# aaryaamoharir/ImageTransformations

Hardware: AMD Instinct MI355X
Metric: Mpixels/sec, 5x5 Gaussian + bilinear rotate on 4K RGB; % HBM roofline (higher is better)
Workload: dtype u8/f32

## Files before the change

imagetransformations_amd/csrc/affine.hip:

```cpp
#include "imgxf_common.h"
#include "pixel_ops.h"
#include <math.h>
#include <algorithm>
#include <string.h>
#include <stdlib.h>

namespace imgxf {

struct AffineParams {
    double m[6];
    int fx[6];
    int64_t q0, q3;
    int64_t q1, q4;
    int64_t x00, y00;
    u32 ntx_magic;
    int sx[4], sy[4];
    u8 fill[4];
    int strip_w;
};

struct FastArith {
    typedef float T;
    static __device__ __forceinline__ T mul(T a, T b) { return a * b; }
    static __device__ __forceinline__ T add(T a, T b) { return a + b; }
// ... 1026 lines not shown

}
#include "affine_mf.inc"
#include "affine_wq.inc"
namespace imgxf {

constexpr int BILINEAR_TALL_NOT_TAKEN = 1 << 30;

template <int BHT, int PITCH, int MAXROWS>
static int launch_bilinear_tall(const View& s, const View& d, const AffineParams& Pin, const View& dbg, const double* m,
                                int bw, int bh, int ntx, bool pr, hipStream_t st) {
    const AffineParams& P = Pin;
    const int bwt = (int)ceil(fabs(m[0]) * 31 + fabs(m[1]) * (BHT - 1)) + 4;
    const int bht = (int)ceil(fabs(m[3]) * 31 + fabs(m[4]) * (BHT - 1)) + 4;
    const int ntyt = (d.h + BHT - 1) / BHT;
    if (bwt > PITCH || bht > MAXROWS || bw > PITCH || (int64_t)ntx * ntyt * ntx >= ((int64_t)1 << 32))
        return BILINEAR_TALL_NOT_TAKEN;
    const bool want_f32 = dbg.p != nullptr;
    const int fpb = knob_int(K_AFFINE_FPB, 16);
    const int afpb = fpb;
    const bool mf = BHT == MF_TILE_H && !want_f32 && afpb >= 2 && d.n >= 2 && bht <= 64 &&
                    (int64_t)d.h * d.rs < ((int64_t)1 << 32);
    const int nch = (bwt * 3 + 15 + 15) / 16;
    const bool dma = mf && !knob_set(K_AFFINE_NO_DMA) && bht <= 52 && bwt <= 52 && 52 * nch <= 768 &&
                     ((((uintptr_t)s.p) | (uintptr_t)s.rs | (uintptr_t)s.fs) & 15) == 0 && s.w * 3 >= 16 &&
                     (int64_t)s.h * s.rs < ((int64_t)1 << 32);
    if (mf && !knob_set(K_AFFINE_NO_DMA)) {
        const int bwq = (int)ceil(fabs(m[0]) * 31 + fabs(m[1]) * 15) + 4, bhq = (int)ceil(fabs(m[3]) * 31 + fabs(m[4]) * 15) + 4;
        const int nchq = (bwq * 3 + 15 + 15) / 16;
        const int ntxq = (d.w + 127) / 128, ntyq = (d.h + 15) / 16;
        const bool aligned = ((((uintptr_t)s.p) | (uintptr_t)s.rs | (uintptr_t)s.fs | ((uintptr_t)d.p) | (uintptr_t)d.rs | (uintptr_t)d.fs) & 15) == 0 &&
                             (d.w * 3) % 16 == 0 && s.w * 3 >= 16;
        if (aligned && bwq <= WQ_PITCH && bhq * nchq <= WQ_MAXCH && bhq * (WQ_PITCH / 4) <= 192 &&
            (int64_t)s.h * s.rs < ((int64_t)1 << 32) && (int64_t)ntxq * ntyq < ((int64_t)1 << 27)) {
            AffineParams Pq = Pin;
            Pq.strip_w = 0;
            const int fpbq = knob_int(K_AFFINE_FPB, 24);
            dim3 grid((unsigned)(ntxq * ntyq), (unsigned)((d.n + fpbq - 1) / fpbq));
            if (ntxq >= 8) { Pq.strip_w = (ntxq + 7) / 8; grid.x = (unsigned)(8 * Pq.strip_w * ntyq); }
            const size_t lds = (size_t)4 * ((size_t)bhq * WQ_PITCH * 4 + 2 * ((size_t)bhq * nchq * 16 + 64)) + 2 * 16 * 384;
            if (pr) hipLaunchKernelGGL((affine_bilinear_wq_kernel<true>), grid, dim3(256), lds, st, s, d, Pq, ntxq, ntyq, fpbq, nchq, bhq);
            else hipLaunchKernelGGL((affine_bilinear_wq_kernel<false>), grid, dim3(256), lds, st, s, d, Pq, ntxq, ntyq, fpbq, nchq, bhq);
            return launch_status();
        }
    }
    if (dma) {
        dim3 grid((unsigned)(ntx * ntyt), (unsigned)((d.n + afpb - 1) / afpb));
        AffineParams Ps = Pin;
        if (ntx >= 16) { Ps.strip_w = (ntx + 7) / 8; grid.x = (unsigned)(8 * Ps.strip_w * ntyt); }
        const size_t lds = (size_t)52 * 56 * 4 + 2 * ((size_t)52 * nch * 16 + 64);
        if (pr) hipLaunchKernelGGL((affine_bilinear_mf_kernel<true, 56, 13, true>), grid, dim3(256), lds, st, s, d, Ps, ntx, ntyt, fpb, nch);
        else hipLaunchKernelGGL((affine_bilinear_mf_kernel<false, 56, 13, true>), grid, dim3(256), lds, st, s, d, Ps, ntx, ntyt, fpb, nch);
        return launch_status();
    }
    TileList list;
    list.n = 0;
    const int64_t ax = 31 * P.q0, bx = (BHT - 1) * P.q1, ay = 31 * P.q3, by = (BHT - 1) * P.q4;
    const int64_t xlo_o = std::min(ax, (int64_t)0) + std::min(bx, (int64_t)0), xhi_o = std::max(ax, (int64_t)0) + std::max(bx, (int64_t)0);
    const int64_t ylo_o = std::min(ay, (int64_t)0) + std::min(by, (int64_t)0), yhi_o = std::max(ay, (int64_t)0) + std::max(by, (int64_t)0);
    for (int ty = 0; ty < ntyt && list.n <= BILINEAR_LIST_MAX; ++ty)
        for (int tx = 0; tx < ntx; ++tx) {
            const int64_t XT = P.x00 + (int64_t)(tx * 32) * P.q0 + (int64_t)(ty * BHT) * P.q1;
            const int64_t YT = P.y00 + (int64_t)(tx * 32) * P.q3 + (int64_t)(ty * BHT) * P.q4;
            const bool clean = (int)((XT + xlo_o) >> 40) >= 0 && (int)((YT + ylo_o) >> 40) >= 0 &&
                               (int)((XT + xhi_o) >> 40) + 1 <= s.w - 1 && (int)((YT + yhi_o) >> 40) + 1 <= s.h - 1 &&
                               tx * 32 + 32 <= d.w && ty * BHT + BHT <= d.h &&
                               !((int)((XT + xhi_o) >> 40) + 1 == s.w - 1 && (int)((YT + yhi_o) >> 40) + 1 == s.h - 1);
            if (!clean) {
                if (list.n < BILINEAR_LIST_MAX) list.idx[list.n] = (u32)(ty * ntx + tx);
                ++list.n;
            }
        }
    if (list.n > BILINEAR_LIST_MAX) return BILINEAR_TALL_NOT_TAKEN;
    if (list.n < ntx * ntyt && mf) {
        const dim3 grid((unsigned)(ntx * ntyt), (unsigned)((d.n + afpb - 1) / afpb));
        const size_t lds = (size_t)2 * PITCH * (bht <= 52 ? 52 : 64) * 4 + 16;
        if (bht <= 52) {
            if (pr) hipLaunchKernelGGL((affine_bilinear_mf_kernel<true, PITCH, 13, false>), grid, dim3(256), lds, st, s, d, P, ntx, ntyt, fpb, 0);
            else hipLaunchKernelGGL((affine_bilinear_mf_kernel<false, PITCH, 13, false>), grid, dim3(256), lds, st, s, d, P, ntx, ntyt, fpb, 0);
        } else {
            if (pr) hipLaunchKernelGGL((affine_bilinear_mf_kernel<true, PITCH, 16, false>), grid, dim3(256), lds, st, s, d, P, ntx, ntyt, fpb, 0);
            else hipLaunchKernelGGL((affine_bilinear_mf_kernel<false, PITCH, 16, false>), grid, dim3(256), lds, st, s, d, P, ntx, ntyt, fpb, 0);
        }
        IMGXF_CHECK(launch_status());
    } else if (list.n < ntx * ntyt) {
        const dim3 grid((unsigned)(ntx * ntyt), (unsigned)d.n);
        const size_t lds = (size_t)PITCH * bht * 4 + 16;
        if (pr && want_f32) hipLaunchKernelGGL((affine_bilinear_lds_interior_kernel<true, PITCH, true, BHT>), grid, dim3(256), lds, st, s, d, P, dbg, ntx, ntyt);
        else if (pr) hipLaunchKernelGGL((affine_bilinear_lds_interior_kernel<true, PITCH, false, BHT>), grid, dim3(256), lds, st, s, d, P, dbg, ntx, ntyt);
        else if (want_f32) hipLaunchKernelGGL((affine_bilinear_lds_interior_kernel<false, PITCH, true, BHT>), grid, dim3(256), lds, st, s, d, P, dbg, ntx, ntyt);
        else hipLaunchKernelGGL((affine_bilinear_lds_interior_kernel<false, PITCH, false, BHT>), grid, dim3(256), lds, st, s, d, P, dbg, ntx, ntyt);
        IMGXF_CHECK(launch_status());
    }
    if (list.n > 0) {
        const dim3 grid((unsigned)((BHT / 32) * list.n), (unsigned)d.n);
        const size_t lds = (size_t)PITCH * bh * 4 + 16;
        if (pr && want_f32) hipLaunchKernelGGL((affine_bilinear_lds_list_kernel<true, PITCH, true, BHT>), grid, dim3(256), lds, st, s, d, P, dbg, ntx, list);
        else if (pr) hipLaunchKernelGGL((affine_bilinear_lds_list_kernel<true, PITCH, false, BHT>), grid, dim3(256), lds, st, s, d, P, dbg, ntx, list);
        else if (want_f32) hipLaunchKernelGGL((affine_bilinear_lds_list_kernel<false, PITCH, true, BHT>), grid, dim3(256), lds, st, s, d, P, dbg, ntx, list);
        else hipLaunchKernelGGL((affine_bilinear_lds_list_kernel<false, PITCH, false, BHT>), grid, dim3(256), lds, st, s, d, P, dbg, ntx, list);
    }
    return launch_status();
}

int run_affine(const imgxf_view* src, const imgxf_view* dst, const double* m, int filter,
               const uint8_t* fill, int precise, const imgxf_view* dbg_f32, void* stream) {
    IMGXF_CHECK(check_view(src));
    IMGXF_CHECK(check_view(dst));
    if (!m) return IMGXF_ERR_NULL;
    if (src->n != dst->n || src->c != dst->c) return IMGXF_ERR_SHAPE;
    if (filter < 0 || filter > 2) return IMGXF_ERR_ARG;
    if (filter == IMGXF_FILTER_NEAREST && m[1] == 0.0 && m[3] == 0.0) return IMGXF_ERR_UNSUPPORTED;
    if (filter != IMGXF_FILTER_NEAREST && src->c == 4) return IMGXF_ERR_UNSUPPORTED;
    if (empty_view(dst)) return IMGXF_OK;
    if (empty_view(src)) return IMGXF_ERR_SHAPE;
    AffineParams P; memset(&P, 0, sizeof(P));
    for (int i = 0; i < 6; ++i) P.m[i] = m[i];
    affine_fixed_matrix(m, P.fx);
    if (fill) for (int j = 0; j < dst->c; ++j) P.fill[j] = fill[j];
    View dbg; memset(&dbg, 0, sizeof(dbg));
    if (dbg_f32) {
        IMGXF_CHECK(check_view(dbg_f32, 4));
        if (!same_geometry(dst, dbg_f32)) return IMGXF_ERR_SHAPE;
        dbg = make_view(dbg_f32);
    }
    const View s = make_view(src), d = make_view(dst);
    hipStream_t st = (hipStream_t)stream;
    const bool pr = precise != 0 || filter == IMGXF_FILTER_NEAREST;
    if (filter == IMGXF_FILTER_NEAREST && src->c == 3 && !knob_set(K_AFFINE_NO_LDS) &&
        ((((uintptr_t)src->data) | (uintptr_t)src->row_stride | (uintptr_t)src->frame_stride) & 3) == 0) {
        bool nowrap = true;
        for (int cy = 0; cy < 2; ++cy)
            for (int cx = 0; cx < 2; ++cx) {
                const double X = cx ? dst->w + 32 : 0, Y = cy ? dst->h + 32 : 0;
                const double xs = (double)P.fx[2] + (double)P.fx[1] * Y + (double)P.fx[0] * X;
                const double ys = (double)P.fx[5] + (double)P.fx[4] * Y + (double)P.fx[3] * X;
                if (fabs(xs) > 2.0e9 || fabs(ys) > 2.0e9) nowrap = false;
            }
        const int bw = (int)ceil((fabs((double)P.fx[0]) * 31 + fabs((double)P.fx[1]) * 31) / 65536.0) + 3;
        const int bh = (int)ceil((fabs((double)P.fx[3]) * 31 + fabs((double)P.fx[4]) * 31) / 65536.0) + 3;
        const int ntx = (d.w + 31) / 32, nty = (d.h + 31) / 32;
        if (nowrap && bw <= 97 && bh <= 100 && (int64_t)ntx * nty < 0x7fffffff && d.n <= 65535) {
            dim3 grid((unsigned)(ntx * nty), (unsigned)d.n);
            P.ntx_magic = (u32)((((uint64_t)1 << 32) + ntx - 1) / ntx);
            const bool no_dma = knob_set(K_AFFINE_NO_DMA);
            {
                const int bwq = (int)ceil((fabs((double)P.fx[0]) * 31 + fabs((double)P.fx[1]) * 15) / 65536.0) + 3;
                const int bhq = (int)ceil((fabs((double)P.fx[3]) * 31 + fabs((double)P.fx[4]) * 15) / 65536.0) + 3;
                const int nchq = (bwq * 3 + 15 + 15) / 16;
                const int kwq = (bhq * nchq + 63) / 64;
                const int ntxq = (d.w + 127) / 128, ntyq = (d.h + 15) / 16;
                const bool aligned = ((((uintptr_t)s.p) | (uintptr_t)s.rs | (uintptr_t)s.fs | ((uintptr_t)d.p) | (uintptr_t)d.rs | (uintptr_t)d.fs) & 15) == 0 &&
                                     (d.w * 3) % 16 == 0 && (s.w * 3) % 16 == 0 && s.w * 3 >= 16 &&
                                     (int64_t)s.h * s.rs < ((int64_t)1 << 32);
                if (aligned && !no_dma && kwq <= NQ_KW && (int64_t)ntxq * ntyq < ((int64_t)1 << 27)) {
                    AffineParams Pq = P;
                    Pq.strip_w = 0;
                    unsigned gx = (unsigned)(ntxq * ntyq);
                    const int fpbq = max(1, min(knob_int(K_AFFINE_FPB, 1), d.n));
                    const dim3 grid(gx, (unsigned)((d.n + fpbq - 1) / fpbq));
                    const size_t nbufq = fpbq > 1 ? 2 : 1;
                    const size_t lds = nbufq * ((size_t)4 * ((size_t)bhq * nchq * 16 + 16) + 16 * 384);
#define IMGXF_NQ_LAUNCH(KWV) hipLaunchKernelGGL((affine_nearest_wq_kernel<KWV>), grid, dim3(256), lds, st, s, d, Pq, ntxq, ntyq, fpbq, nchq, bhq)
                    switch (kwq) {
                        case 1: IMGXF_NQ_LAUNCH(1); break; case 2: IMGXF_NQ_LAUNCH(2); break; case 3: IMGXF_NQ_LAUNCH(3); break;
                        case 4: IMGXF_NQ_LAUNCH(4); break; case 5: IMGXF_NQ_LAUNCH(5); break; case 6: IMGXF_NQ_LAUNCH(6); break;
                        case 7: IMGXF_NQ_LAUNCH(7); break; default: IMGXF_NQ_LAUNCH(8); break;
                    }
#undef IMGXF_NQ_LAUNCH
                    return launch_status();
                }
            }
            if (bw <= 49 && bh <= 52 && !no_dma && src->w * 3 >= 16 && (src->w * 3) % 16 == 0 &&
                ((((uintptr_t)src->data) | (uintptr_t)src->row_stride | (uintptr_t)src->frame_stride) & 15) == 0) {
                const int bw64 = (int)ceil((fabs((double)P.fx[0]) * 31 + fabs((double)P.fx[1]) * 63) / 65536.0) + 3;
                const int bh64 = (int)ceil((fabs((double)P.fx[3]) * 31 + fabs((double)P.fx[4]) * 63) / 65536.0) + 3;
                const bool no_tall = knob_set(K_AFFINE_NO_TALL);
                if (bw64 <= 64 && bh64 <= 80 && !no_tall) {
                    const int nty64 = (d.h + 63) / 64;
                    unsigned gx = (unsigned)(ntx * nty64);
                    if (ntx >= 16) { P.strip_w = (ntx + 7) / 8; gx = (unsigned)(8 * P.strip_w * nty64); }
                    hipLaunchKernelGGL((affine_nearest_dma_kernel<64, 13>), dim3(gx, (unsigned)d.n), dim3(256),
                                       (size_t)13 * 16 * bh64 + 32, st, s, d, P, ntx, nty64);
                } else {
                    hipLaunchKernelGGL((affine_nearest_dma_kernel<32, 11>), grid, dim3(256), (size_t)11 * 16 * bh + 32, st, s, d, P, ntx, nty);
                }
                return launch_status();
            }
            if (bw <= 49) hipLaunchKernelGGL((affine_nearest_lds_kernel<49>), grid, dim3(256), (size_t)49 * bh * 4 + 16, st, s, d, P, ntx, nty);
            else if (bw <= 65) hipLaunchKernelGGL((affine_nearest_lds_kernel<65>), grid, dim3(256), (size_t)65 * bh * 4 + 16, st, s, d, P, ntx, nty);
            else hipLaunchKernelGGL((affine_nearest_lds_kernel<97>), grid, dim3(256), (size_t)97 * bh * 4 + 16, st, s, d, P, ntx, nty);
            return launch_status();
        }
    }
    bool fixed_ok = fabs(m[0]) < 64.0 && fabs(m[3]) < 64.0;
    for (int cy = 0; cy < 2 && fixed_ok; ++cy)
        for (int cx = 0; cx < 2; ++cx) {
            const double X = (cx ? dst->w + 4 : 0) + 0.5, Y = (cy ? dst->h : 0) + 0.5;
            const double xs = m[0] * X + m[1] * Y + m[2], ys = m[3] * X + m[4] * Y + m[5];
            if (!(fabs(xs) < 2097152.0 && fabs(ys) < 2097152.0)) fixed_ok = false;
        }
    P.q0 = fixed_ok ? llround(m[0] * 1099511627776.0) : 0;
    P.q3 = fixed_ok ? llround(m[3] * 1099511627776.0) : 0;
    fixed_ok = fixed_ok && fabs(m[1]) < 64.0 && fabs(m[4]) < 64.0;
    P.q1 = fixed_ok ? llround(m[1] * 1099511627776.0) : 0;
    P.q4 = fixed_ok ? llround(m[4] * 1099511627776.0) : 0;
    for (int k = 0; k < 4; ++k) {
        P.sx[k] = (int)((k * P.q0 + (k * P.q0 >= 0 ? 32768 : -32768)) / 65536);
        P.sy[k] = (int)((k * P.q3 + (k * P.q3 >= 0 ? 32768 : -32768)) / 65536);
    }
    if (fixed_ok) {
        const double x0d = (m[0] * 0.5 + m[1] * 0.5) + m[2] - 0.5, y0d = (m[3] * 0.5 + m[4] * 0.5) + m[5] - 0.5;
        P.x00 = (int64_t)floor(x0d * 1099511627776.0);
        P.y00 = (int64_t)floor(y0d * 1099511627776.0);
    }
    if (filter == IMGXF_FILTER_BILINEAR && (src->c == 1 || src->c == 3) && src->w >= 3 && src->h >= 2 && fixed_ok) {
        const bool no_lds = knob_set(K_AFFINE_NO_LDS);
        if (src->c == 3 && !no_lds &&
            ((((uintptr_t)src->data) | (uintptr_t)src->row_stride | (uintptr_t)src->frame_stride) & 3) == 0) {
            const int bw = (int)ceil(fabs(m[0]) * 31 + fabs(m[1]) * 31) + 4;
            const int bh = (int)ceil(fabs(m[3]) * 31 + fabs(m[4]) * 31) + 4;
            const int ntx = (d.w + 31) / 32, nty = (d.h + 31) / 32;
            if (bw <= 97 && bh <= 100 && (int64_t)ntx * nty < 0x7fffffff && d.n <= 65535) {
                dim3 grid((unsigned)(ntx * nty), (unsigned)d.n);
                P.ntx_magic = (u32)((((uint64_t)1 << 32) + ntx - 1) / ntx);
#define IMGXF_LDS_LAUNCH(KERNEL, PITCH, GRID, NTY, LDSB)                                            \
    do {                                                                                           \
        if (dbg.p) {                                                                               \
            if (pr) hipLaunchKernelGGL((KERNEL<true, PITCH, true>), GRID, dim3(256), LDSB, st, s, d, P, dbg, ntx, NTY); \
            else hipLaunchKernelGGL((KERNEL<false, PITCH, true>), GRID, dim3(256), LDSB, st, s, d, P, dbg, ntx, NTY); \
        } else {                                                                                   \
            if (pr) hipLaunchKernelGGL((KERNEL<true, PITCH, false>), GRID, dim3(256), LDSB, st, s, d, P, dbg, ntx, NTY); \
            else hipLaunchKernelGGL((KERNEL<false, PITCH, false>), GRID, dim3(256), LDSB, st, s, d, P, dbg, ntx, NTY); \
        }                                                                                          \
    } while (0)
#define IMGXF_LDS(PITCH)                                                                           \
    do {                                                                                           \
        const size_t lds = (size_t)PITCH * bh * 4 + 16;                                            \
        IMGXF_LDS_LAUNCH(affine_bilinear_lds_kernel, PITCH, grid, nty, lds);                       \
        return launch_status();                                                                    \
    } while (0)
                const bool no_tall = knob_set(K_AFFINE_NO_TALL);
                if (!no_tall) {
                    const int rc = launch_bilinear_tall<64, 49, 64>(s, d, P, dbg, m, bw, bh, ntx, pr, st);
                    if (rc != BILINEAR_TALL_NOT_TAKEN) return rc;
                }
                if (bw <= 49) IMGXF_LDS(49);
                if (bw <= 65) IMGXF_LDS(65);
                IMGXF_LDS(97);
#undef IMGXF_LDS
#undef IMGXF_LDS_LAUNCH
            }
        }
#define IMGXF_BIL(CC, PR, TXG, WX)                                                                 \
    do {                                                                                           \
        constexpr int BW = WX * TXG * 4, BH = (4 / WX) * (64 / TXG);                               \
        const int ntx = (d.w + BW - 1) / BW, nty = (d.h + BH - 1) / BH;                            \
        const int64_t nb = (int64_t)ntx * nty * d.n;                                               \
        if (nb > 0x7fffffff) return IMGXF_ERR_SHAPE;                                               \
        hipLaunchKernelGGL((affine_bilinear_kernel<CC, PR, TXG, WX>), dim3((unsigned)nb), dim3(256), 0, st, \
                           s, d, P, dbg, ntx, nty, (int)nb);                                       \
        return launch_status();                                                                    \
    } while (0)
        if (src->c == 3) {
            if (pr) IMGXF_BIL(3, true, 8, 2); else IMGXF_BIL(3, false, 8, 2);
        } else {
            if (pr) IMGXF_BIL(1, true, 8, 2); else IMGXF_BIL(1, false, 8, 2);
        }
#undef IMGXF_BIL
    }
    {
        const bool no_shear = knob_set(K_AFFINE_NO_SHEAR_FAST);
        const bool honly = m[3] == 0.0 && m[4] == 1.0 && m[5] == floor(m[5]) && fabs(m[5]) < 1.0e9;
        if (filter == IMGXF_FILTER_BICUBIC && honly && src->c == 3 && !dbg.p && !no_shear && src->w >= 4) {
            dim3 block(256), grid((unsigned)((d.w + 1023) / 1024), (unsigned)d.h, (unsigned)d.n);
            if (m[0] == 1.0) {
                if (pr) hipLaunchKernelGGL((shear_bicubic_kernel<true, true>), grid, block, 0, st, s, d, P);
                else hipLaunchKernelGGL((shear_bicubic_kernel<false, true>), grid, block, 0, st, s, d, P);
                IMGXF_CHECK(launch_status());
                hipLaunchKernelGGL(shear_edges_kernel, dim3((unsigned)((d.h * 8 + 255) / 256), (unsigned)d.n), dim3(256), 0, st, s, d, P);
                return launch_status();
            }
            if (pr) hipLaunchKernelGGL((shear_bicubic_kernel<true, false>), grid, block, 0, st, s, d, P);
            else hipLaunchKernelGGL((shear_bicubic_kernel<false, false>), grid, block, 0, st, s, d, P);
            return launch_status();
        }
    }
    switch (src->c) {
        case 1: return pr ? launch_affine_filter<1, PreciseArith>(filter, s, d, P, dbg, st)
                          : launch_affine_filter<1, FastArith>(filter, s, d, P, dbg, st);
        case 3: return pr ? launch_affine_filter<3, PreciseArith>(filter, s, d, P, dbg, st)
                          : launch_affine_filter<3, FastArith>(filter, s, d, P, dbg, st);
        case 4: return launch_affine_filter<4, PreciseArith>(filter, s, d, P, dbg, st);
        default: return IMGXF_ERR_UNSUPPORTED;
    }
}

__global__ void scale_tables_kernel(int* xtab, int* ytab, int* meta, int ow, int oh, int sw, int sh,
                                    double a0, double a2, double a4, double a5) {
    if (threadIdx.x == 0 && blockIdx.x == 0) {
        double xo = __dadd_rn(a2, __dmul_rn(a0, 0.5));
        int xmin = ow, xmax = 0;
        for (int x = 0; x < ow; ++x) {
            const int xin = xo < 0.0 ? -1 : (int)xo;
            if (xin >= 0 && xin < sw) {
                xmax = x + 1;
                if (x < xmin) xmin = x;
// ... 126 lines not shown
```

imagetransformations_amd/csrc/affine_wq.inc:

```
#pragma once

namespace imgxf {

constexpr int WQ_PITCH = 28;
constexpr int WQ_MAXCH = 192;

template <bool PRECISE>
__global__ __launch_bounds__(256, 3) void affine_bilinear_wq_kernel(View s, View d, AffineParams P, int ntx, int nty, int fpb,
                                                                   int nch, int rows) {
    constexpr int C = 3, SW = 32, BH = 16, BW = 4 * SW, PITCH = WQ_PITCH, NG = PITCH / 4;
    constexpr float GUARDP = 4.0f / 32768.0f;
    constexpr u32 GTOP = 8u << 17;
    constexpr int FONE = 1 << 24, FHALF = 1 << 23, CG32 = 1 << 6;
    extern __shared__ __attribute__((aligned(16))) u32 wq_lds[];
    const int orig = blockIdx.x, xcd = orig & 7, l = orig >> 3;
    int tyb, txb;
    if (P.strip_w) { tyb = l / P.strip_w; txb = xcd * P.strip_w + (l - tyb * P.strip_w); }
    else { const int nb = ntx * nty, q = nb >> 3, r = nb & 7;
           const int logical = (xcd < r ? xcd * (q + 1) : r * (q + 1) + (xcd - r) * q) + l;
           tyb = logical / ntx; txb = logical - tyb * ntx; }
    if (txb >= ntx || tyb >= nty) return;
    const int lane = threadIdx.x & 63, wave = __builtin_amdgcn_readfirstlane(threadIdx.x >> 6);
    const int f_begin = blockIdx.y * fpb, f_end = min(d.n, f_begin + fpb);
    const int sx0 = txb * BW + wave * SW, sy0 = tyb * BH;
    const bool wave_in = sx0 < d.w;

    const u32 pk_bytes = (u32)(rows * nch * 16 + 64);
    const u32 wave_bytes = (u32)(rows * PITCH * 4) + 2u * pk_bytes;
    u32* const srct = wq_lds + wave * (wave_bytes / 4);
    u32* const slots = wq_lds + 4 * (wave_bytes / 4);

    const int64_t XT = P.x00 + (int64_t)sx0 * P.q0 + (int64_t)sy0 * P.q1;
    const int64_t YT = P.y00 + (int64_t)sx0 * P.q3 + (int64_t)sy0 * P.q4;
    const int64_t ax = (SW - 1) * P.q0, bx = (BH - 1) * P.q1, ay = (SW - 1) * P.q3, by = (BH - 1) * P.q4;
    const int64_t xlo = XT + min(ax, (int64_t)0) + min(bx, (int64_t)0), xhi = XT + max(ax, (int64_t)0) + max(bx, (int64_t)0);
    const int64_t ylo = YT + min(ay, (int64_t)0) + min(by, (int64_t)0), yhi = YT + max(ay, (int64_t)0) + max(by, (int64_t)0);
    const int ux_lo = __builtin_amdgcn_readfirstlane((int)(xlo >> 40)), uy_lo = __builtin_amdgcn_readfirstlane((int)(ylo >> 40));
    const int sx_hi = __builtin_amdgcn_readfirstlane((int)(xhi >> 40) + 1), sy_hi = __builtin_amdgcn_readfirstlane((int)(yhi >> 40) + 1);
    const bool interior = ux_lo >= 0 && uy_lo >= 0 && sx_hi <= s.w - 1 && sy_hi <= s.h - 1 && sx0 + SW <= d.w && sy0 + BH <= d.h;

    const int lx = (lane & 7) * 4, x0 = sx0 + lx;
    u32 la[8];
    float w00[8], w01[8], w10[8], w11[8];
    u32 cneed = 0, fillm = 0, okm = 0;
#pragma unroll
    for (int half = 0; half < 2; ++half) {
        const int ly = half * 8 + (lane >> 3);
        const int64_t XL = XT + lx * P.q0 + ly * P.q1 - ((int64_t)ux_lo << 40);
        const int64_t YL = YT + lx * P.q3 + ly * P.q4 - ((int64_t)uy_lo << 40);
        const int Xb = (int)((XL + 32768) >> 16), Yb = (int)((YL + 32768) >> 16);
#pragma unroll
        for (int j = 0; j < 4; ++j) {
            const int k = half * 4 + j;
            const int X32 = Xb + P.sx[j], Y32 = Yb + P.sy[j];
            const u32 fx = (u32)X32 & (FONE - 1), fy = (u32)Y32 & (FONE - 1);
            const float dx = (float)fx * 5.9604644775390625e-08f, dy = (float)fy * 5.9604644775390625e-08f;
            const float ox = 1.0f - dx, oy = 1.0f - dy;
            w00[k] = ox * oy; w01[k] = dx * oy; w10[k] = ox * dy; w11[k] = dx * dy;
            la[k] = (u32)(((Y32 >> 24) * PITCH + (X32 >> 24)) * 4);
            const u32 gx = ((u32)X32 + CG32) & (FONE - 1), gy = ((u32)Y32 + CG32) & (FONE - 1);
            cneed |= (min(gx, gy) < 2u * CG32) ? 1u << k : 0u;
            if (!interior) {
                const int xi = (X32 >> 24) + ux_lo, yi = (Y32 >> 24) + uy_lo;
                const bool valid = x0 + j < d.w && sy0 + ly < d.h;
                const bool sure = (((fx & (FHALF - 1)) - CG32) < (u32)(FHALF - 2 * CG32)) &&
                                  (((fy & (FHALF - 1)) - CG32) < (u32)(FHALF - 2 * CG32));
                const bool inner = valid && sure && xi >= 0 && xi + 1 <= s.w - 1 && yi >= 0 && yi + 1 <= s.h - 1;
                const bool far_out = valid && sure && (xi < -1 || xi > s.w || yi < -1 || yi > s.h);
                if (!inner) { w00[k] = 0.0f; w01[k] = 0.0f; w10[k] = 0.0f; w11[k] = 0.0f; la[k] = 0u; }
                cneed = (cneed & ~(1u << k)) | ((valid && !inner && !far_out) ? 1u << k : 0u);
                fillm |= far_out ? 1u << k : 0u;
                okm |= valid ? 1u << k : 0u;
            }
        }
    }
    if (interior) okm = 0xffu;

    const int a0 = (ux_lo * 3) & ~15, e0 = ux_lo * 3 - a0;
    const u32 rgbx_bytes = (u32)(rows * PITCH * 4);
    const u32 pk_base = (u32)(uintptr_t)(__attribute__((address_space(3))) u32*)srct + rgbx_bytes;
    u32 dma_off[3];
    bool dma_ok[3];
    u32 ex_rd[3], ex_wr[3];
    bool ex_ok[3];
    {
        const u32 lim = (u32)(((int64_t)(s.h - 1) * s.rs + (int64_t)s.w * 3 - 16) & ~(int64_t)15);
#pragma unroll
        for (int i = 0; i < 3; ++i) {
            const int c = i * 64 + lane;
            const int row = c / nch, ch = c - row * nch;
            dma_ok[i] = c < rows * nch && wave_in;
            const int64_t go = (int64_t)clampi(uy_lo + row, 0, s.h - 1) * s.rs + a0 + 16 * ch;
            dma_off[i] = (u32)min(max(go, (int64_t)0), (int64_t)lim);
        }
#pragma unroll
        for (int it = 0; it < 3; ++it) {
            const int u = lane + 64 * it;
            const int rr = u / NG, t = u - rr * NG;
            ex_ok[it] = u < rows * NG;
            ex_rd[it] = (u32)(rr * nch * 16 + ((e0 + 12 * t) & ~3));
            ex_wr[it] = (u32)((rr * PITCH + 4 * t) * 4);
        }
    }
    const int kw = (rows * nch + 63) / 64;
    auto dma_issue = [&](int f, int pbuf) {
        const u8* fb = s.p + (int64_t)f * s.fs;
#pragma unroll
        for (int i = 0; i < 3; ++i) {
            const u32 ldst = __builtin_amdgcn_readfirstlane(pk_base + (u32)pbuf * pk_bytes + (u32)(i * 1024));
            if (i < kw && dma_ok[i]) glds16_hidden(fb, dma_off[i], ldst);
        }
    };
    auto expand = [&](int pbuf) {
        const char* pk = (const char*)srct + rgbx_bytes + pbuf * pk_bytes;
        const u32 sh = (u32)(e0 & 3);
#pragma unroll
        for (int it = 0; it < 3; ++it) {
            if (!ex_ok[it]) continue;
            const u32* q = (const u32*)(pk + ex_rd[it]);
            const u32 d0 = q[0], d1 = q[1], d2 = q[2], d3 = q[3];
            const u32 a = __builtin_amdgcn_alignbyte(d1, d0, sh), b = __builtin_amdgcn_alignbyte(d2, d1, sh);
            const u32 c = __builtin_amdgcn_alignbyte(d3, d2, sh);
            uint4 o;
            o.x = a; o.y = __builtin_amdgcn_alignbyte(b, a, 3u); o.z = __builtin_amdgcn_alignbyte(c, b, 2u); o.w = c >> 8;
            *(uint4*)((char*)srct + ex_wr[it]) = o;
        }
    };

    auto put_pixel = [&](u32 (&od)[2][3], int k, u32 val) {
        const int half = k >> 2, j = k & 3;
        u32 o0 = half ? od[1][0] : od[0][0], o1 = half ? od[1][1] : od[0][1], o2 = half ? od[1][2] : od[0][2];
        if (j == 0) o0 = (o0 & 0xff000000u) | val;
        else if (j == 1) { o0 = (o0 & 0x00ffffffu) | (val << 24); o1 = (o1 & 0xffff0000u) | (val >> 8); }
        else if (j == 2) { o1 = (o1 & 0x0000ffffu) | (val << 16); o2 = (o2 & 0xffffff00u) | (val >> 16); }
        else o2 = (o2 & 0x000000ffu) | (val << 8);
        if (half) { od[1][0] = o0; od[1][1] = o1; od[1][2] = o2; } else { od[0][0] = o0; od[0][1] = o1; od[0][2] = o2; }
    };

    auto slow_pixels = [&](u32 need, int f, u32 (&od)[2][3]) {
        const u8* sp = s.p + (int64_t)f * s.fs;
#pragma unroll 1
        for (u32 m = need; m; m &= m - 1) {
            const int k = __builtin_ctz(m), half = k >> 2, j = k & 3;
            const int y = sy0 + half * 8 + (lane >> 3);
            const bool unsure = (cneed >> k) & 1u;
            u32 val = 0;
            bool have = true;
            const double xc = (double)(x0 + j) + 0.5, yc = (double)y + 0.5;
            double xin = (P.m[0] * xc + P.m[1] * yc) + P.m[2];
            double yin = (P.m[3] * xc + P.m[4] * yc) + P.m[5];
            if (unsure && !(xin >= 0.0 && xin < (double)s.w && yin >= 0.0 && yin < (double)s.h)) {
                val = (u32)P.fill[0] | ((u32)P.fill[1] << 8) | ((u32)P.fill[2] << 16);
            } else {
                xin -= 0.5; yin -= 0.5;
                const double xfl = floor(xin), yfl = floor(yin);
                const int xq = (int)xfl, yq = (int)yfl;
                const double dxd = xin - xfl, dyd = yin - yfl;
                u32 p00, p01, p10, p11;
                if (unsure) {
                    const int xa = clampi(xq, 0, s.w - 1) * C, xb = clampi(xq + 1, 0, s.w - 1) * C;
                    const u8* r0 = sp + (int64_t)clampi(yq, 0, s.h - 1) * s.rs;
                    const bool has1 = (yq + 1 >= 0) && (yq + 1 < s.h);
                    const u8* r1 = has1 ? sp + (int64_t)(yq + 1) * s.rs : r0;
                    p00 = (u32)r0[xa] | ((u32)r0[xa + 1] << 8) | ((u32)r0[xa + 2] << 16);
                    p01 = (u32)r0[xb] | ((u32)r0[xb + 1] << 8) | ((u32)r0[xb + 2] << 16);
                    p10 = (u32)r1[xa] | ((u32)r1[xa + 1] << 8) | ((u32)r1[xa + 2] << 16);
                    p11 = (u32)r1[xb] | ((u32)r1[xb + 1] << 8) | ((u32)r1[xb + 2] << 16);
                } else {
                    const u32* tp = srct + (yq - uy_lo) * PITCH + (xq - ux_lo);
                    p00 = tp[0]; p01 = tp[1]; p10 = tp[PITCH]; p11 = tp[PITCH + 1];
                    have = (((p00 ^ p01) | (p10 ^ p11) | (p00 ^ p10)) << 8) != 0;
                }
#pragma unroll
                for (int c = 0; c < C; ++c) {
                    const double ta = (double)((p00 >> (8 * c)) & 0xffu), tb = (double)((p01 >> (8 * c)) & 0xffu);
                    const double tc = (double)((p10 >> (8 * c)) & 0xffu), te = (double)((p11 >> (8 * c)) & 0xffu);
                    const double w1 = ta + (tb - ta) * dxd, w2 = tc + (te - tc) * dxd;
                    const double w = w1 + (w2 - w1) * dyd;
                    val |= (u32)(u8)(int)w << (8 * c);
                }
            }
            if (have) put_pixel(od, k, val);
        }
    };

    auto gather_frame = [&](int f, u32* slot) {
        const u32 boff = (u32)(uintptr_t)(__attribute__((address_space(3))) const u32*)srct;
        u32 od[2][3] = {{0u, 0u, 0u}, {0u, 0u, 0u}};
        u32 need = cneed;
#pragma unroll
        for (int half = 0; half < 2; ++half) {
            if (half) __builtin_amdgcn_sched_barrier(0);
            u32 tq[4][3], mq[4];
#pragma unroll
            for (int j = 0; j < 4; ++j) {
                const int k = half * 4 + j;
                const u32* tp = (const u32*)(__attribute__((address_space(3))) const u32*)(uintptr_t)(boff + la[k]);
                const u32 p00 = tp[0], p01 = tp[1], p10 = tp[PITCH], p11 = tp[PITCH + 1];
                constexpr float X0 = PRECISE ? 256.0f + GUARDP : 0.0f;
                float v[3];
                v[0] = fmaf(w00[k], tapf<0>(p00), X0); v[1] = fmaf(w00[k], tapf<1>(p00), X0); v[2] = fmaf(w00[k], tapf<2>(p00), X0);
                v[0] = fmaf(w01[k], tapf<0>(p01), v[0]); v[1] = fmaf(w01[k], tapf<1>(p01), v[1]); v[2] = fmaf(w01[k], tapf<2>(p01), v[2]);
                v[0] = fmaf(w10[k], tapf<0>(p10), v[0]); v[1] = fmaf(w10[k], tapf<1>(p10), v[1]); v[2] = fmaf(w10[k], tapf<2>(p10), v[2]);
                v[0] = fmaf(w11[k], tapf<0>(p11), v[0]); v[1] = fmaf(w11[k], tapf<1>(p11), v[1]); v[2] = fmaf(w11[k], tapf<2>(p11), v[2]);
                if (PRECISE) {
#pragma unroll
                    for (int c = 0; c < 3; ++c) tq[j][c] = __builtin_amdgcn_alignbit(__float_as_uint(v[c]), __float_as_uint(v[c]), 15u);
                    mq[j] = min(min(tq[j][0], tq[j][1]), tq[j][2]);
                } else {
                    u32 (&o)[3] = od[half];
#pragma unroll
                    for (int c = 0; c < 3; ++c) {
                        const int bpos = j * 3 + c;
                        o[bpos >> 2] = __builtin_amdgcn_cvt_pk_u8_f32(floorf(v[c]), bpos & 3, o[bpos >> 2]);
                    }
                }
            }
            if (PRECISE) {
                constexpr u32 PAIR = 0x0c0c0400u, QUAD = 0x05040100u;
                const u32 a0 = __builtin_amdgcn_perm(tq[0][1], tq[0][0], PAIR), a1 = __builtin_amdgcn_perm(tq[1][0], tq[0][2], PAIR);
                const u32 a2 = __builtin_amdgcn_perm(tq[1][2], tq[1][1], PAIR), a3 = __builtin_amdgcn_perm(tq[2][1], tq[2][0], PAIR);
                const u32 a4 = __builtin_amdgcn_perm(tq[3][0], tq[2][2], PAIR), a5 = __builtin_amdgcn_perm(tq[3][2], tq[3][1], PAIR);
                od[half][0] = __builtin_amdgcn_perm(a1, a0, QUAD);
                od[half][1] = __builtin_amdgcn_perm(a3, a2, QUAD);
                od[half][2] = __builtin_amdgcn_perm(a5, a4, QUAD);
                const u32 mg = min(min(mq[0], mq[1]), min(mq[2], mq[3]));
                if (__builtin_amdgcn_ballot_w64(mg < GTOP) != 0) {
#pragma unroll
                    for (int j = 0; j < 4; ++j) need |= (mq[j] < GTOP) ? 1u << (half * 4 + j) : 0u;
                }
            }
        }
        need &= okm & ~fillm;
        if (need) slow_pixels(need, f, od);
        if (fillm && ((u32)P.fill[0] | (u32)P.fill[1] | (u32)P.fill[2])) {
            const u32 val = (u32)P.fill[0] | ((u32)P.fill[1] << 8) | ((u32)P.fill[2] << 16);
#pragma unroll 1
            for (u32 m = fillm; m; m &= m - 1) put_pixel(od, __builtin_ctz(m), val);
        }
#pragma unroll
        for (int half = 0; half < 2; ++half) {
            u32* ws = slot + (half * 8 + (lane >> 3)) * 96 + wave * 24 + (lane & 7) * 3;
            ws[0] = od[half][0]; ws[1] = od[half][1]; ws[2] = od[half][2];
        }
    };

    const int rb16 = (int)((int64_t)d.w * C / 16);
    auto flush = [&](int f, const u32* slot) {
        u8* dframe = d.p + (int64_t)f * d.fs;
#pragma unroll
        for (int pass = 0; pass < 2; ++pass) {
            const int ch = pass * 64 + lane;
            const int r = wave * 4 + ch / 24, ck = ch - (ch / 24) * 24;
            if (ch < 96 && sy0 + r < d.h && txb * 24 + ck < rb16) {
                const uint4 o4 = *(const uint4*)(slot + r * 96 + ck * 4);
                *(uint4*)(dframe + (int64_t)(sy0 + r) * d.rs + (int64_t)txb * (BW * C) + ck * 16) = o4;
            }
        }
    };

    if (wave_in) { dma_issue(f_begin, 0); if (f_begin + 1 < f_end) dma_issue(f_begin + 1, 1); }
    int pb = 0;
#pragma unroll 1
    for (int f = f_begin; f < f_end; ++f) {
        u32* slot = slots + ((f - f_begin) & 1) * (16 * 96);
        if (wave_in) {
            if (f + 1 >= f_end) asm volatile("s_waitcnt vmcnt(0)" ::: "memory");
            else if (kw == 1) asm volatile("s_waitcnt vmcnt(1)" ::: "memory");
            else if (kw == 2) asm volatile("s_waitcnt vmcnt(2)" ::: "memory");
            else asm volatile("s_waitcnt vmcnt(3)" ::: "memory");
        }
        if (f > f_begin) flush(f - 1, slots + ((f - 1 - f_begin) & 1) * (16 * 96));
        if (wave_in) {
            expand(pb);
            asm volatile("s_waitcnt lgkmcnt(0)" ::: "memory");
            if (f + 2 < f_end) dma_issue(f + 2, pb);
            gather_frame(f, slot);
            pb ^= 1;
        }
        asm volatile("s_waitcnt lgkmcnt(0)\n\ts_barrier" ::: "memory");
    }
    flush(f_end - 1, slots + ((f_end - 1 - f_begin) & 1) * (16 * 96));
}

constexpr int NQ_KW = 8;

template <int KWT>
__device__ __forceinline__ void nq_wait() {
    static_assert(KWT >= 0 && KWT <= NQ_KW, "");
    if constexpr (KWT == 0) asm volatile("s_waitcnt vmcnt(0)" ::: "memory");
    else if constexpr (KWT == 1) asm volatile("s_waitcnt vmcnt(1)" ::: "memory");
    else if constexpr (KWT == 2) asm volatile("s_waitcnt vmcnt(2)" ::: "memory");
    else if constexpr (KWT == 3) asm volatile("s_waitcnt vmcnt(3)" ::: "memory");
    else if constexpr (KWT == 4) asm volatile("s_waitcnt vmcnt(4)" ::: "memory");
    else if constexpr (KWT == 5) asm volatile("s_waitcnt vmcnt(5)" ::: "memory");
    else if constexpr (KWT == 6) asm volatile("s_waitcnt vmcnt(6)" ::: "memory");
    else if constexpr (KWT == 7) asm volatile("s_waitcnt vmcnt(7)" ::: "memory");
    else asm volatile("s_waitcnt vmcnt(8)" ::: "memory");
}

template <int KW>
__global__ __launch_bounds__(256) void affine_nearest_wq_kernel(View s, View d, AffineParams P, int ntx, int nty, int fpb,
                                                                int nch, int rows) {
    constexpr int C = 3, SW = 32, BH = 16, BW = 4 * SW;
    extern __shared__ __attribute__((aligned(16))) u32 nq_lds[];
    const int orig = blockIdx.x, xcd = orig & 7, l = orig >> 3;
    int tyb, txb;
    if (P.strip_w) { tyb = l / P.strip_w; txb = xcd * P.strip_w + (l - tyb * P.strip_w); }
    else { const int nb = ntx * nty, q = nb >> 3, r = nb & 7;
           const int logical = (xcd < r ? xcd * (q + 1) : r * (q + 1) + (xcd - r) * q) + l;
           tyb = logical / ntx; txb = logical - tyb * ntx; }
    if (txb >= ntx || tyb >= nty) return;
    const int lane = threadIdx.x & 63, wave = __builtin_amdgcn_readfirstlane(threadIdx.x >> 6);
    const int f_begin = blockIdx.y * fpb, f_end = min(d.n, f_begin + fpb);
    const int sx0 = txb * BW + wave * SW, sy0 = tyb * BH;
    const int dpitch = nch * 16;
    const u32 box_bytes = (u32)(rows * dpitch + 16);
    const u32 nbuf = fpb > 1 ? 2u : 1u;
    char* const boxes = (char*)nq_lds + wave * (nbuf * box_bytes);
    u32* const slots = nq_lds + 4 * (nbuf * box_bytes) / 4;

    const int XT = P.fx[2] + P.fx[1] * sy0 + P.fx[0] * sx0;
    const int YT = P.fx[5] + P.fx[4] * sy0 + P.fx[3] * sx0;
    const int ax = (SW - 1) * P.fx[0], bx = (BH - 1) * P.fx[1], ay = (SW - 1) * P.fx[3], by = (BH - 1) * P.fx[4];
    const int sx_lo = max((XT + min(ax, 0) + min(bx, 0)) >> 16, 0), sx_hi = min((XT + max(ax, 0) + max(bx, 0)) >> 16, s.w - 1);
    const int sy_lo = max((YT + min(ay, 0) + min(by, 0)) >> 16, 0), sy_hi = min((YT + max(ay, 0) + max(by, 0)) >> 16, s.h - 1);
    const int bwc = sx_hi - sx_lo + 1, bhc = sy_hi - sy_lo + 1;
    const bool wave_in = sx0 < d.w && bwc > 0 && bhc > 0;
    const int a0 = (sx_lo * 3) & ~15;
    const int last_chunk = s.w * 3 - 16;

    const u32 fillw = (u32)P.fill[0] | ((u32)P.fill[1] << 8) | ((u32)P.fill[2] << 16);
    const int lx = (lane & 7) * 4;
    u32 bo[8];
    u32 inm = 0;
#pragma unroll
    for (int half = 0; half < 2; ++half) {
        const int ly = half * 8 + (lane >> 3);
        const int XL = XT + lx * P.fx[0] + ly * P.fx[1], YL = YT + lx * P.fx[3] + ly * P.fx[4];
#pragma unroll
        for (int j = 0; j < 4; ++j) {
            const int xi = ((XL + j * P.fx[0]) >> 16) - sx_lo, yi = ((YL + j * P.fx[3]) >> 16) - sy_lo;
            const bool in = wave_in && (u32)xi < (u32)bwc && (u32)yi < (u32)bhc;
            bo[half * 4 + j] = in ? (u32)(yi * dpitch + (xi + sx_lo) * 3 - a0) : 0u;
            inm |= in ? 1u << (half * 4 + j) : 0u;
        }
    }

    u32 dma_off[KW];
    bool dma_ok[KW];
#pragma unroll
    for (int i = 0; i < KW; ++i) {
        const int c = i * 64 + lane;
        const int row = c / nch, ch = c - row * nch;
        dma_ok[i] = wave_in && c < rows * nch;
        dma_off[i] = (u32)((int64_t)min(sy_lo + row, s.h - 1) * s.rs + min(a0 + ch * 16, last_chunk));
    }
    const u32 box_base = (u32)(uintptr_t)(__attribute__((address_space(3))) char*)boxes;
    auto dma_issue = [&](int f, int pbuf) {
        const u8* fb = s.p + (int64_t)f * s.fs;
#pragma unroll
        for (int i = 0; i < KW; ++i) {
            const u32 ldst = __builtin_amdgcn_readfirstlane(box_base + (u32)pbuf * box_bytes + (u32)(i * 1024));
            if (dma_ok[i]) glds16_hidden(fb, dma_off[i], ldst);
        }
    };
    auto gather_frame = [&](int pbuf, u32* slot) {
        const char* box = boxes + pbuf * box_bytes;
#pragma unroll
        for (int half = 0; half < 2; ++half) {
            u32 px[4];
#pragma unroll
            for (int j = 0; j < 4; ++j) {
                const int k = half * 4 + j;
                const u32* wp = (const u32*)(box + (bo[k] & ~3u));
                const u32 lo = wp[0], hi = wp[1];
                const u32 t = __builtin_amdgcn_alignbyte(hi, lo, bo[k] & 3u);
                px[j] = ((inm >> k) & 1u) ? (t & 0xffffffu) : fillw;
            }
            u32* ws = slot + (half * 8 + (lane >> 3)) * 96 + wave * 24 + (lane & 7) * 3;
            ws[0] = px[0] | (px[1] << 24);
            ws[1] = (px[1] >> 8) | (px[2] << 16);
            ws[2] = (px[2] >> 16) | (px[3] << 8);
        }
    };
    const int rb16 = (int)((int64_t)d.w * C / 16);
    auto flush = [&](int f, const u32* slot) {
        u8* dframe = d.p + (int64_t)f * d.fs;
#pragma unroll
        for (int pass = 0; pass < 2; ++pass) {
            const int ch = pass * 64 + lane;
            const int r = wave * 4 + ch / 24, ck = ch - (ch / 24) * 24;
            if (ch < 96 && sy0 + r < d.h && txb * 24 + ck < rb16) {
                const uint4 o4 = *(const uint4*)(slot + r * 96 + ck * 4);
                *(uint4*)(dframe + (int64_t)(sy0 + r) * d.rs + (int64_t)txb * (BW * C) + ck * 16) = o4;
            }
        }
    };

    dma_issue(f_begin, 0);
    if (f_begin + 1 < f_end) dma_issue(f_begin + 1, 1);
#pragma unroll 1
    for (int f = f_begin; f < f_end; ++f) {
        const int it = f - f_begin;
        if (f + 1 >= f_end) nq_wait<0>(); else nq_wait<KW>();
        if (it) flush(f - 1, slots + ((it - 1) & 1) * (16 * 96));
        gather_frame(it & 1, slots + (it & 1) * (16 * 96));
        asm volatile("s_waitcnt lgkmcnt(0)" ::: "memory");
        if (f + 2 < f_end) dma_issue(f + 2, it & 1);
        asm volatile("s_barrier" ::: "memory");
    }
    flush(f_end - 1, slots + ((f_end - 1 - f_begin) & 1) * (16 * 96));
}

}
```

Baseline: 368,300.

## Skip source DMA for fully-out-of-bounds waves and precompute output store addresses

In the bilinear WQ kernel, waves whose pixels all map outside the source (fill-only) no longer issue source DMA loads or run the gather. They just park zero/fill output into the LDS slot. Output store offsets and predicates are now computed once per block instead of every frame, and frame pointers advance incrementally. The vmcnt wait accounts for outstanding stores, and a 32-bit destination-size guard was added. Both kernels share the new flush helper.

```diff
diff --git a/imagetransformations_amd/csrc/affine.hip b/imagetransformations_amd/csrc/affine.hip
--- a/imagetransformations_amd/csrc/affine.hip
+++ b/imagetransformations_amd/csrc/affine.hip
@@ -1202,7 +1202,7 @@
                 const int ntxq = (d.w + 127) / 128, ntyq = (d.h + 15) / 16;
                 const bool aligned = ((((uintptr_t)s.p) | (uintptr_t)s.rs | (uintptr_t)s.fs | ((uintptr_t)d.p) | (uintptr_t)d.rs | (uintptr_t)d.fs) & 15) == 0 &&
                                      (d.w * 3) % 16 == 0 && (s.w * 3) % 16 == 0 && s.w * 3 >= 16 &&
-                                     (int64_t)s.h * s.rs < ((int64_t)1 << 32);
+                                     (int64_t)s.h * s.rs < ((int64_t)1 << 32) && (int64_t)d.h * d.rs < ((int64_t)1 << 32);
                 if (aligned && !no_dma && kwq <= NQ_KW && (int64_t)ntxq * ntyq < ((int64_t)1 << 27)) {
                     AffineParams Pq = P;
                     Pq.strip_w = 0;
diff --git a/imagetransformations_amd/csrc/affine_wq.inc b/imagetransformations_amd/csrc/affine_wq.inc
--- a/imagetransformations_amd/csrc/affine_wq.inc
+++ b/imagetransformations_amd/csrc/affine_wq.inc
@@ -4,6 +4,50 @@
 
 constexpr int WQ_PITCH = 28;
 constexpr int WQ_MAXCH = 192;
+constexpr u32 WQ_SLOT = 16 * 96;
+
+struct WqStores {
+    u32 rd[2];
+    u32 wr[2];
+    bool ok[2];
+    bool any[2];
+    int n;
+};
+
+__device__ __forceinline__ WqStores wq_stores_setup(const View& d, int txb, int sy0, int wave, int lane) {
+    WqStores S;
+    const int rb16 = (int)((int64_t)d.w * 3 / 16);
+    S.n = 0;
+#pragma unroll
+    for (int pass = 0; pass < 2; ++pass) {
+        const int ch = pass * 64 + lane;
+        const int r = wave * 4 + ch / 24, ck = ch - (ch / 24) * 24;
+        S.ok[pass] = ch < 96 && sy0 + r < d.h && txb * 24 + ck < rb16;
+        S.any[pass] = __builtin_amdgcn_ballot_w64(S.ok[pass]) != 0;
+        S.rd[pass] = (u32)(r * 96 + ck * 4);
+        S.wr[pass] = S.ok[pass] ? (u32)((int64_t)(sy0 + r) * d.rs + (int64_t)txb * 384 + ck * 16) : 0u;
+        S.n += S.any[pass] ? 1 : 0;
+    }
+    return S;
+}
+
+__device__ __forceinline__ void wq_flush(const WqStores& S, const u32* slot, u8* dframe) {
+#pragma unroll
+    for (int pass = 0; pass < 2; ++pass) {
+        if (S.any[pass]) {
+            if (S.ok[pass]) *(uint4*)(dframe + S.wr[pass]) = *(const uint4*)(slot + S.rd[pass]);
+        }
+    }
+}
+
+template <int N>
+__device__ __forceinline__ void wq_vmcnt() { asm volatile("s_waitcnt vmcnt(%0)" :: "n"(N) : "memory"); }
+__device__ __forceinline__ void wq_wait_vm(int n) {
+    switch (n) {
+        case 0: wq_vmcnt<0>(); break; case 1: wq_vmcnt<1>(); break; case 2: wq_vmcnt<2>(); break;
+        case 3: wq_vmcnt<3>(); break; case 4: wq_vmcnt<4>(); break; default: wq_vmcnt<5>(); break;
+    }
+}
 
 template <bool PRECISE>
 __global__ __launch_bounds__(256, 3) void affine_bilinear_wq_kernel(View s, View d, AffineParams P, int ntx, int nty, int fpb,
@@ -75,6 +119,8 @@
         }
     }
     if (interior) okm = 0xffu;
+    const bool wave_far = !interior && __builtin_amdgcn_ballot_w64((okm & ~fillm) != 0) == 0;
+    const bool wave_src = wave_in && !wave_far;
 
     const int a0 = (ux_lo * 3) & ~15, e0 = ux_lo * 3 - a0;
     const u32 rgbx_bytes = (u32)(rows * PITCH * 4);
@@ -89,7 +135,7 @@
         for (int i = 0; i < 3; ++i) {
             const int c = i * 64 + lane;
             const int row = c / nch, ch = c - row * nch;
-            dma_ok[i] = c < rows * nch && wave_in;
+            dma_ok[i] = c < rows * nch && wave_src;
             const int64_t go = (int64_t)clampi(uy_lo + row, 0, s.h - 1) * s.rs + a0 + 16 * ch;
             dma_off[i] = (u32)min(max(go, (int64_t)0), (int64_t)lim);
         }
@@ -103,8 +149,7 @@
         }
     }
     const int kw = (rows * nch + 63) / 64;
-    auto dma_issue = [&](int f, int pbuf) {
-        const u8* fb = s.p + (int64_t)f * s.fs;
+    auto dma_issue = [&](const u8* fb, int pbuf) {
 #pragma unroll
         for (int i = 0; i < 3; ++i) {
             const u32 ldst = __builtin_amdgcn_readfirstlane(pk_base + (u32)pbuf * pk_bytes + (u32)(i * 1024));
@@ -137,8 +182,7 @@
         if (half) { od[1][0] = o0; od[1][1] = o1; od[1][2] = o2; } else { od[0][0] = o0; od[0][1] = o1; od[0][2] = o2; }
     };
 
-    auto slow_pixels = [&](u32 need, int f, u32 (&od)[2][3]) {
-        const u8* sp = s.p + (int64_t)f * s.fs;
+    auto slow_pixels = [&](u32 need, const u8* sp, u32 (&od)[2][3]) {
 #pragma unroll 1
         for (u32 m = need; m; m &= m - 1) {
             const int k = __builtin_ctz(m), half = k >> 2, j = k & 3;
@@ -184,7 +228,20 @@
         }
     };
 
-    auto gather_frame = [&](int f, u32* slot) {
+    auto park = [&](u32 (&od)[2][3], u32* slot) {
+        if (fillm && ((u32)P.fill[0] | (u32)P.fill[1] | (u32)P.fill[2])) {
+            const u32 val = (u32)P.fill[0] | ((u32)P.fill[1] << 8) | ((u32)P.fill[2] << 16);
+#pragma unroll 1
+            for (u32 m = fillm; m; m &= m - 1) put_pixel(od, __builtin_ctz(m), val);
+        }
+#pragma unroll
+        for (int half = 0; half < 2; ++half) {
+            u32* ws = slot + (half * 8 + (lane >> 3)) * 96 + wave * 24 + (lane & 7) * 3;
+            ws[0] = od[half][0]; ws[1] = od[half][1]; ws[2] = od[half][2];
+        }
+    };
+
+    auto gather_frame = [&](const u8* sp, u32* slot) {
         const u32 boff = (u32)(uintptr_t)(__attribute__((address_space(3))) const u32*)srct;
         u32 od[2][3] = {{0u, 0u, 0u}, {0u, 0u, 0u}};
         u32 need = cneed;
@@ -232,55 +289,37 @@
             }
         }
         need &= okm & ~fillm;
-        if (need) slow_pixels(need, f, od);
-        if (fillm && ((u32)P.fill[0] | (u32)P.fill[1] | (u32)P.fill[2])) {
-            const u32 val = (u32)P.fill[0] | ((u32)P.fill[1] << 8) | ((u32)P.fill[2] << 16);
-#pragma unroll 1
-            for (u32 m = fillm; m; m &= m - 1) put_pixel(od, __builtin_ctz(m), val);
-        }
-#pragma unroll
-        for (int half = 0; half < 2; ++half) {
-            u32* ws = slot + (half * 8 + (lane >> 3)) * 96 + wave * 24 + (lane & 7) * 3;
-            ws[0] = od[half][0]; ws[1] = od[half][1]; ws[2] = od[half][2];
-        }
-    };
-
-    const int rb16 = (int)((int64_t)d.w * C / 16);
-    auto flush = [&](int f, const u32* slot) {
-        u8* dframe = d.p + (int64_t)f * d.fs;
-#pragma unroll
-        for (int pass = 0; pass < 2; ++pass) {
-            const int ch = pass * 64 + lane;
-            const int r = wave * 4 + ch / 24, ck = ch - (ch / 24) * 24;
-            if (ch < 96 && sy0 + r < d.h && txb * 24 + ck < rb16) {
-                const uint4 o4 = *(const uint4*)(slot + r * 96 + ck * 4);
-                *(uint4*)(dframe + (int64_t)(sy0 + r) * d.rs + (int64_t)txb * (BW * C) + ck * 16) = o4;
-            }
-        }
-    };
-
-    if (wave_in) { dma_issue(f_begin, 0); if (f_begin + 1 < f_end) dma_issue(f_begin + 1, 1); }
+        if (need) slow_pixels(need, sp, od);
+        park(od, slot);
+    };
+
+    const WqStores S = wq_stores_setup(d, txb, sy0, wave, lane);
+
+    const u8* sframe = s.p + (int64_t)f_begin * s.fs;
+    u8* dframe = d.p + (int64_t)f_begin * d.fs;
+    const int64_t sfs = s.fs, dfs = d.fs;
+    if (wave_src) { dma_issue(sframe, 0); if (f_begin + 1 < f_end) dma_issue(sframe + sfs, 1); }
     int pb = 0;
+    u32 cur = 0;
 #pragma unroll 1
     for (int f = f_begin; f < f_end; ++f) {
-        u32* slot = slots + ((f - f_begin) & 1) * (16 * 96);
-        if (wave_in) {
-            if (f + 1 >= f_end) asm volatile("s_waitcnt vmcnt(0)" ::: "memory");
-            else if (kw == 1) asm volatile("s_waitcnt vmcnt(1)" ::: "memory");
-            else if (kw == 2) asm volatile("s_waitcnt vmcnt(2)" ::: "memory");
-            else asm volatile("s_waitcnt vmcnt(3)" ::: "memory");
-        }
-        if (f > f_begin) flush(f - 1, slots + ((f - 1 - f_begin) & 1) * (16 * 96));
-        if (wave_in) {
+        if (wave_src) wq_wait_vm(f + 1 >= f_end ? 0 : f - f_begin >= 2 ? kw + S.n : kw);
+        if (f > f_begin) { wq_flush(S, slots + (cur ^ WQ_SLOT), dframe); dframe += dfs; }
+        if (wave_src) {
             expand(pb);
             asm volatile("s_waitcnt lgkmcnt(0)" ::: "memory");
-            if (f + 2 < f_end) dma_issue(f + 2, pb);
-            gather_frame(f, slot);
+            if (f + 2 < f_end) dma_issue(sframe + 2 * sfs, pb);
+            gather_frame(sframe, slots + cur);
             pb ^= 1;
+        } else if (wave_in) {
+            u32 od[2][3] = {{0u, 0u, 0u}, {0u, 0u, 0u}};
+            park(od, slots + cur);
         }
         asm volatile("s_waitcnt lgkmcnt(0)\n\ts_barrier" ::: "memory");
-    }
-    flush(f_end - 1, slots + ((f_end - 1 - f_begin) & 1) * (16 * 96));
+        sframe += sfs;
+        cur ^= WQ_SLOT;
+    }
+    wq_flush(S, slots + (cur ^ WQ_SLOT), dframe);
 }
 
 constexpr int NQ_KW = 8;
@@ -302,7 +341,7 @@
 template <int KW>
 __global__ __launch_bounds__(256) void affine_nearest_wq_kernel(View s, View d, AffineParams P, int ntx, int nty, int fpb,
                                                                 int nch, int rows) {
-    constexpr int C = 3, SW = 32, BH = 16, BW = 4 * SW;
+    constexpr int SW = 32, BH = 16, BW = 4 * SW;
     extern __shared__ __attribute__((aligned(16))) u32 nq_lds[];
     const int orig = blockIdx.x, xcd = orig & 7, l = orig >> 3;
     int tyb, txb;
@@ -384,19 +423,7 @@
             ws[2] = (px[2] >> 16) | (px[3] << 8);
         }
     };
-    const int rb16 = (int)((int64_t)d.w * C / 16);
-    auto flush = [&](int f, const u32* slot) {
-        u8* dframe = d.p + (int64_t)f * d.fs;
-#pragma unroll
-        for (int pass = 0; pass < 2; ++pass) {
-            const int ch = pass * 64 + lane;
-            const int r = wave * 4 + ch / 24, ck = ch - (ch / 24) * 24;
-            if (ch < 96 && sy0 + r < d.h && txb * 24 + ck < rb16) {
-                const uint4 o4 = *(const uint4*)(slot + r * 96 + ck * 4);
-                *(uint4*)(dframe + (int64_t)(sy0 + r) * d.rs + (int64_t)txb * (BW * C) + ck * 16) = o4;
-            }
-        }
-    };
+    const WqStores S = wq_stores_setup(d, txb, sy0, wave, lane);
 
     dma_issue(f_begin, 0);
     if (f_begin + 1 < f_end) dma_issue(f_begin + 1, 1);
@@ -404,13 +431,13 @@
     for (int f = f_begin; f < f_end; ++f) {
         const int it = f - f_begin;
         if (f + 1 >= f_end) nq_wait<0>(); else nq_wait<KW>();
-        if (it) flush(f - 1, slots + ((it - 1) & 1) * (16 * 96));
-        gather_frame(it & 1, slots + (it & 1) * (16 * 96));
+        if (it) wq_flush(S, slots + ((it - 1) & 1) * WQ_SLOT, d.p + (int64_t)(f - 1) * d.fs);
+        gather_frame(it & 1, slots + (it & 1) * WQ_SLOT);
         asm volatile("s_waitcnt lgkmcnt(0)" ::: "memory");
         if (f + 2 < f_end) dma_issue(f + 2, it & 1);
         asm volatile("s_barrier" ::: "memory");
     }
-    flush(f_end - 1, slots + ((f_end - 1 - f_begin) & 1) * (16 * 96));
-}
-
-}
+    wq_flush(S, slots + ((f_end - 1 - f_begin) & 1) * WQ_SLOT, d.p + (int64_t)(f_end - 1) * d.fs);
+}
+
+}
```

Result: no change. 370,400 (median of 5 runs) (+0.6%).
